# ALVI-Labs/frankenstein

Hardware: AMD Instinct MI355X
Metric: neural frames/sec (train fwd+bwd+AdamW, whole job) (higher is better)
Workload: dtype bf16; 1 GPU; brainformer-small (6L d=384 6x64 heads, N=6144 tokens) + 2-block perceiver, L1 head; fwd+bwd+clip+AdamW; per_gpu_batch=32, global_batch=32, frames_T=600, electrodes=256, parallelism=dp1, weights=random-init (seed 42)

## Files before the change

frankenstein_amd/_lib.py:

```python
from __future__ import annotations

import ctypes as C
from pathlib import Path

import os

LIB_PATH = Path(os.environ.get("FRANKEN_HIP_LIB") or Path(__file__).resolve().parent / "libfranken_hip.so")

FK_F32, FK_BF16 = 0, 1
MASK_NONE, MASK_CAUSAL, MASK_BLOCK_CAUSAL, MASK_PREFIX, MASK_KEYPAD, MASK_DENSE = 0, 1, 2, 3, 4, 5
NORM_LAYER, NORM_RMS = 0, 1
ATTN_Q_PRESCALED = 1
GEMV_GELU = 1
NT_RING2, NT_RING192, NT_RING128, NT_BIG, NT_GLDS4, NT_GLDS, NT_STAGED = range(7)
NT_ROUTE_F32 = -2
ATTN_FWD_GENERIC, ATTN_FWD_FEWQ, ATTN_FWD_PS, ATTN_FWD_ASM = range(4)
ATTN_DQ_GENERIC, ATTN_DQ_FEWQ, ATTN_DQ_PS, ATTN_DQ_ASM = range(4)
ATTN_DKDV_GENERIC, ATTN_DKDV_PS, ATTN_DKDV_ASM, ATTN_DKDVW_ASM = range(4)

_p, _i64, _int, _f32, _f64, _sz, _u32 = C.c_void_p, C.c_int64, C.c_int, C.c_float, C.c_double, C.c_size_t, C.c_uint32

SIGNATURES = {
    "fk_version": (_int, []),
    "fk_last_error": (C.c_char_p, []),
    "fk_gemm_nt": (_int, [_p, _i64, _p, _i64, _p, _i64, _i64, _i64, _i64, _p, _p, _i64, _i64, _int, _int, _p]),
    "fk_gemv_nt": (_int, [_p, _i64, _p, _i64, _p, _i64, _i64, _i64, _i64, _p, _p, _i64, _p, _p, _f32, _int, _int, _int, _p]),
    "fk_gemm_nt_rope": (_int, [_p, _i64, _p, _i64, _p, _i64, _i64, _i64, _i64, _p, _p, _i64, _i64, _i64, _i64, _i64, _i64, _i64, _int, _p]),
    "fk_gemm_nt_swiglu": (_int, [_p, _i64, _p, _i64, _p, _i64, _p, _i64, _i64, _i64, _i64, _int, _p]),
    "fk_gemm_nt_dswiglu": (_int, [_p, _i64, _p, _i64, _p, _i64, _p, _i64, _i64, _i64, _i64, _int, _p]),
    "fk_mlp_bwd_fused": (_int, [_p, _i64, _p, _i64, _p, _i64, _p, _i64, _p, _i64, _p, _i64, _i64, _i64, _i64, _int, _p]),
    "fk_gemm_nt_route": (_int, [_i64, _i64, _i64, _int, _int, _int, _int]),
    "fk_gemm_tn_route": (_int, [_i64, _i64, _i64, _int, _p, _p]),
    "fk_gemm_tn_workspace_bytes": (_sz, [_i64, _i64, _i64, _int]),
    "fk_gemm_tn": (_int, [_p, _i64, _p, _i64, _p, _i64, _i64, _i64, _i64, _int, _int, _p, _sz, _p]),
    "fk_gemm_tn_swiglu": (_int, [_p, _i64, _p, _i64, _p, _p, _i64, _i64, _i64, _i64, _int, _p, _sz, _p]),
    "fk_colsum_workspace_bytes": (_sz, [_i64, _i64]),
    "fk_colsum": (_int, [_p, _i64, _p, _i64, _i64, _int, _int, _p, _sz, _p]),
    "fk_attn_fwd": (_int, [_p, _p, _p, _p, _p] + [_i64] * 13 + [_int, _i64, _i64, _i64, _p, _p, _f32, _int, _int, _p]),
    "fk_attn_bwd": (_int, [_p] * 10 + [_i64] * 13 + [_int, _i64, _i64, _i64, _p, _p, _f32, _p, _i64, _i64, _int, _int, _p]),
    "fk_attn_fwd_dropout": (_int, [_p, _p, _p, _p, _p] + [_i64] * 13 + [_int, _i64, _i64, _i64, _p, _p, _f32, _int, _f32, _p, _u32, _int, _p]),
    "fk_attn_bwd_dropout": (_int, [_p] * 10 + [_i64] * 13 + [_int, _i64, _i64, _i64, _p, _p, _f32, _p, _i64, _i64, _int, _f32, _p, _u32, _int, _p]),
    "fk_attn_route": (_int, [_i64, _i64, _i64, _int, _int, _i64, _i64, _i64, _int, _int, _int, _p, _p, _p]),
    "fk_dropout": (_int, [_p, _p, _p, _i64, _f32, _p, _u32, _int, _p]),
    "fk_norm_fwd": (_int, [_p, _p, _p, _p, _p, _p, _i64, _i64, _f32, _int, _int, _p]),
    "fk_norm_bwd_workspace_bytes": (_sz, [_i64, _i64]),
    "fk_norm_bwd": (_int, [_p] * 9 + [_i64, _i64, _int, _int, _int, _p, _sz, _p]),
    "fk_rope": (_int, [_p, _i64, _i64, _i64, _i64, _i64, _p, _i64, _i64, _int, _int, _p]),
    "fk_patchify": (_int, [_p, _p, _i64, _i64, _i64, _i64, _i64, _int, _p]),
    "fk_swiglu_fwd": (_int, [_p, _p, _i64, _i64, _int, _p]),
    "fk_swiglu_bwd": (_int, [_p, _p, _p, _i64, _i64, _int, _p]),
    "fk_gelu_fwd": (_int, [_p, _p, _i64, _int, _p]),
    "fk_gelu_bwd": (_int, [_p, _p, _p, _i64, _int, _p]),
    "fk_cast_pack": (_int, [_p, _i64, _p, _i64, _i64, _i64, _int, _int, _p]),
    "fk_cast_pack_rows": (_int, [_p, _i64, _p, _i64, _i64, _i64, _int, _i64, _i64, _i64, _int, _p]),
    "fk_cast_pack_multi": (_int, [_p, _i64, _i64, _int, _p]),
    "fk_cast": (_int, [_p, _int, _p, _int, _i64, _p]),
    "fk_add": (_int, [_p, _p, _p, _i64, _int, _p]),
    "fk_gather_rows": (_int, [_p, _i64, _int, _p, _i64, _p, _i64, _int, _i64, _i64, _i64, _int, _p]),
    "fk_scatter_add_rows": (_int, [_p, _int, _p, _i64, _p, _i64, _i64, _p]),
    "fk_prefix_mask": (_int, [_p, _p, _i64, _p, _p, _i64, _i64, _i64, _p]),
    "fk_copy2d": (_int, [_p, _i64, _p, _i64, _i64, _i64, _int, _p]),
    "fk_attn_combine": (_int, [_p, _p, _p, _p, _i64, _i64, _i64, _i64, _i64, _int, _p]),
    "fk_add2d": (_int, [_p, _i64, _p, _i64, _i64, _i64, _p]),
    "fk_gpt_embed_step": (_int, [_p, _p, _p, _p, _p, _i64, _i64, _i64, _int, _p]),
    "fk_kv_append": (_int, [_p, _p, _p, _i64, _i64, _i64, _int, _p]),
    "fk_attn_decode": (_int, [_p, _i64, _p, _i64, _i64, _p, _i64, _p, _i64, _i64, _i64, _f32, _int, _p]),
    "fk_sample_topk": (_int, [_p, _i64, _i64, _i64, _f32, _i64, _p, _p, _p, _p, _p, _i64, _i64, _p, _p]),
    "fk_attn_decode_beam": (_int, [_p, _i64, _p, _i64, _i64, _p, _i64, _p, _i64, _p, _i64, _i64, _i64, _f32, _int, _p]),
    "fk_beam_topk": (_int, [_p, _i64, _i64, _i64, _f32, _i64, _p, _p, _p]),
    "fk_beam_select": (_int, [_p, _p, _i64, _i64, _i64, _p, _p, _p, _p, _p, _p, _p, _p, _i64, _p, _i64, _p]),
    "fk_attn_decode_beam_grouped": (_int, [_p, _i64, _p, _i64, _i64, _i64, _p, _i64, _p, _i64, _p, _i64, _i64, _i64, _i64, _f32, _int, _int, _p]),
    "fk_beam_select_grouped": (_int, [_p, _p, _i64, _i64, _i64, _i64, _i64, _p, _p, _p, _p, _p, _p, _p, _p, _i64, _p, _i64, _p, _p]),
    "fk_beam_select_eos": (_int, [_p, _p, _i64, _i64, _i64, _i64, _i64, _p, _p, _p, _p, _p, _p, _p, _p, _i64, _p, _i64, _p, _i64, _p, _p, _p, _i64, _p, _p, _p]),
    "fk_beam_backtrack": (_int, [_p, _p, _i64, _i64, _i64, _p, _p, _p, _p, _i64, _p, _i64, _i64, _i64, _i64, _p, _p, _p]),
    "fk_sample_topk_eos": (_int, [_p, _i64, _i64, _i64, _f32, _i64, _p, _p, _p, _p, _p, _i64, _i64, _p, _i64, _p, _p, _p, _p, _p]),
# ... 82 lines not shown
```

frankenstein_amd/csrc/attention.hip:

```cpp
#include "fk_common.h"
#include <type_traits>

namespace {

constexpr int NT = 256;
constexpr int BQ = 128;
constexpr int BKV = 64;
constexpr float LOG2E = 1.4426950408889634f;

struct AttnArgs {
  const void *Q, *K, *V, *O, *dO;
  void *Out, *dQ, *dK, *dV;
  float *LSE, *delta;
  int64_t q_bs, q_rs, k_bs, k_rs, v_bs, v_rs, o_bs, o_rs;
  int B, H, Nq, Nk;
  int mask_kind, mask_c, q_off, k_off;
  float scale;
  const float* rope_table; int64_t rope_bs; int rope_off;
  const int* limits; const int* qfirst;
  int flags;
  const unsigned* drop_seed; unsigned drop_site, drop_thresh; float drop_scale;
};

template <typename T, int D> struct AT {
// ... 696 lines not shown
    }
    const char* kt = buf + (i & 1) * FEWQ_TILE;
    const char* vt = kt + FEWQ_BK * 128;
    const int kb = (wave + FEWQ_NW * i) * FEWQ_BK;
    f32x16 sc, dp;
#pragma unroll
    for (int r = 0; r < 16; ++r) { sc[r] = 0.0f; dp[r] = 0.0f; }
#pragma unroll
    for (int s = 0; s < 4; ++s) {
      Frag<T> kf, vf;
      img_row<T, D>(kf, kt, li, s, lh);
      img_row<T, D>(vf, vt, li, s, lh);
      mma32<T>(sc, kf, qf[s]);
      mma32<T>(dp, vf, gf[s]);
    }
    const bool ragged = kb + FEWQ_BK > p.Nk;
#pragma unroll
    for (int r = 0; r < 16; ++r) {
      float pv = __builtin_amdgcn_exp2f(sc[r] * c - lse2);
      if (ragged && kb + acc_row(r, lh) >= p.Nk) pv = 0.0f;
      sc[r] = pv * (dp[r] - dl);
    }
#pragma unroll
    for (int s = 0; s < 2; ++s) {
      Frag<T> df;
      frag_from_acc<T>(df, sc, s);
#pragma unroll
      for (int dt = 0; dt < 2; ++dt) {
        Frag<T> ktf;
        img_tr<T, D>(ktf, kt, 0, s, 32 * dt, lane);
        mma32<T>(dq[dt], ktf, df);
      }
    }
  }
  __syncthreads();
  float* area = reinterpret_cast<float*>(smem);
  {
    float* mine = area + wave * 32 * 64;
#pragma unroll
    for (int dt = 0; dt < 2; ++dt)
#pragma unroll
      for (int r = 0; r < 16; ++r) mine[(dt * 16 + r) * 64 + lane] = dq[dt][r];
  }
  __syncthreads();
  if (wave != 0) return;
#pragma unroll 1
  for (int w = 1; w < FEWQ_NW; ++w) {
    const float* theirs = area + w * 32 * 64;
#pragma unroll
    for (int dt = 0; dt < 2; ++dt)
#pragma unroll
      for (int r = 0; r < 16; ++r) dq[dt][r] += theirs[(dt * 16 + r) * 64 + lane];
  }
  T* dQp = head_ptr<T, D>(p.dQ, p.q_bs, b, hd);
  store_rows_T<T, D>(dQp, p.q_rs, qrow, q_ok, dq, p.scale, lh);
}

template <bool DMA> FK_DEV void tile_sync() {
  if constexpr (DMA) asm volatile("s_waitcnt vmcnt(0) lgkmcnt(0)\n\ts_barrier" ::: "memory");
  else __syncthreads();
}
template <typename T, int D>
__global__ __launch_bounds__(NT) void attn_bwd_dq_kernel(AttnArgs p) {
  using C = AT<T, D>;
  extern __shared__ __attribute__((aligned(16))) char smem[];
  constexpr int IMG = BKV * C::RSTRIDE;
// ... 1482 lines not shown
                        float drop_p, const uint32_t* drop_seed, uint32_t drop_site, int dtype, void* stream) {
  const int64_t st[8] = {q_bs, q_rs, k_bs, k_rs, v_bs, v_rs, o_bs, o_rs};
  int rc = check_common("fk_attn_bwd", B, H, Nq, Nk, D, dtype, mask_kind, mask_c, st, 8);
  if (rc) return rc;
  rc = check_flags_tables("fk_attn_bwd", D, dtype, mask_kind, q_off, k_off, limits, qfirst, flags);
  if (rc) return rc;
  FK_CHECK_ARG(Q && K && V && O && dO && LSE && dQ && dK && dV && delta_ws, "fk_attn_bwd: null pointer");
  FK_CHECK_ARG((((uintptr_t)Q | (uintptr_t)K | (uintptr_t)V | (uintptr_t)O | (uintptr_t)dO | (uintptr_t)dQ | (uintptr_t)dK | (uintptr_t)dV) & 15) == 0,
               "fk_attn_bwd: pointers must be 16-byte aligned");
  AttnArgs a{};
  a.Q = Q; a.K = K; a.V = V; a.O = O; a.dO = dO; a.LSE = const_cast<float*>(LSE); a.delta = delta_ws;
  a.dQ = dQ; a.dK = dK; a.dV = dV;
  fill_common(a, st, B, H, Nq, Nk, mask_kind, mask_c, q_off, k_off, limits, qfirst, scale, flags);
  FK_CHECK_ARG(!rope_table || (Nq == Nk && D % 4 == 0 && ((uintptr_t)rope_table & 15) == 0), "fk_attn_bwd: fused inverse RoPE needs self-attention (Nq == Nk)");
  a.rope_table = rope_table; a.rope_bs = rope_bs; a.rope_off = (int)rope_off;
  rc = set_dropout("fk_attn_bwd", a, drop_p, drop_seed, drop_site, flags);
  if (rc) return rc;
  FK_ATTN_DISPATCH(launch_bwd, a, (hipStream_t)stream);
  FK_CHECK_LAUNCH("fk_attn_bwd");
  return FK_OK;
}

int fk_attn_bwd(const void* Q, const void* K, const void* V, const void* O, const void* dO, const float* LSE,
                void* dQ, void* dK, void* dV, float* delta_ws, int64_t B, int64_t H, int64_t Nq, int64_t Nk, int64_t D,
                int64_t q_bs, int64_t q_rs, int64_t k_bs, int64_t k_rs, int64_t v_bs, int64_t v_rs, int64_t o_bs,
                int64_t o_rs, int mask_kind, int64_t mask_c, int64_t q_off, int64_t k_off, const int32_t* limits,
                const int32_t* qfirst, float scale, const float* rope_table, int64_t rope_bs, int64_t rope_off, int flags,
                int dtype, void* stream) {
  return fk_attn_bwd_dropout(Q, K, V, O, dO, LSE, dQ, dK, dV, delta_ws, B, H, Nq, Nk, D, q_bs, q_rs, k_bs, k_rs, v_bs, v_rs, o_bs, o_rs,
                             mask_kind, mask_c, q_off, k_off, limits, qfirst, scale, rope_table, rope_bs, rope_off, flags, 0.0f, nullptr, 0,
                             dtype, stream);
}

int fk_attn_route(int64_t Nq, int64_t Nk, int64_t D, int dtype, int mask_kind, int64_t mask_c, int64_t q_off, int64_t k_off, int flags,
                  int has_dropout, int has_rope, int* fwd, int* dq, int* dkdv) {
  const int64_t st[1] = {0};
  int rc = check_common("fk_attn_route", 1, 1, Nq, Nk, D, dtype, mask_kind, mask_c, st, 0);
  if (rc) return rc;
  FK_CHECK_ARG((flags & ~FK_ATTN_Q_PRESCALED) == 0 && (!(flags & FK_ATTN_Q_PRESCALED) || (dtype == FK_BF16 && D == 64)),
               "fk_attn_route: bad flags %d (FK_ATTN_Q_PRESCALED needs bf16, D = 64)", flags);
  FK_CHECK_ARG(!(flags & FK_ATTN_Q_PRESCALED) || (mask_kind != FK_MASK_DENSE && !has_dropout),
               "fk_attn_route: dense masks and dropout run on the generic kernels (no FK_ATTN_Q_PRESCALED)");
  FK_CHECK_ARG(!has_rope || Nq == Nk, "fk_attn_route: fused inverse RoPE needs self-attention (Nq == Nk)");
  AttnArgs a{};
  a.Nq = (int)Nq; a.Nk = (int)Nk; a.mask_kind = mask_kind; a.mask_c = (int)mask_c; a.q_off = (int)q_off; a.k_off = (int)k_off;
  a.flags = flags; a.drop_thresh = has_dropout ? 1u : 0u;
  static_assert(Img<bf16_t, 64>::SWZ && !Img<bf16_t, 32>::SWZ && !Img<bf16_t, 128>::SWZ && !Img<float, 64>::SWZ, "the swizzled image: bf16, D = 64");
  const AttnRoute r = attn_route(a, dtype == FK_BF16 && D == 64, has_rope != 0);
  if (fwd) *fwd = r.fwd;
  if (dq) *dq = r.dq;
  if (dkdv) *dkdv = r.dkdv;
  return FK_OK;
}

}
```

frankenstein_amd/engine.py:

```python
from __future__ import annotations

from typing import List, Optional, Sequence, Tuple

import math
import os
import weakref

import torch

from . import kernels as K
from .kernels import NO_MASK

Tensor = torch.Tensor

_COMPUTE_DTYPE = torch.bfloat16
_EPOCH = 0


def set_compute_dtype(dtype) -> None:
    global _COMPUTE_DTYPE
    if isinstance(dtype, str):
        dtype = {"bf16": torch.bfloat16, "bfloat16": torch.bfloat16, "fp32": torch.float32, "float32": torch.float32}[dtype]
    assert dtype in (torch.bfloat16, torch.float32)
    _COMPUTE_DTYPE = dtype
# ... 424 lines not shown
class CrossAttnBranch(torch.autograd.Function):

    @staticmethod
    def forward(ctx, x, context, ln_w, ln_b, qw, kw, vw, pw, spec):
        H, D, mask, eps = spec
        B, T, d = x.shape
        Nc = context.shape[1]
        HD = H * D
        x2, c2 = x.view(B * T, d), context.view(B * Nc, d)
        h, mean, rstd = K.norm_fwd(x2, ln_w.detach(), ln_b.detach(), eps)
        ctx.ln_b = ln_b
        q = K.gemm_nt(h, shadow([qw]))
        kv = K.gemm_nt(c2, shadow([kw, vw]))
        kv3 = kv.view(B, Nc, 2 * HD)
        o, lse = K.attn_fwd(q.view(B, T, H, D), kv3[..., :HD].unflatten(-1, (H, D)), kv3[..., HD:].unflatten(-1, (H, D)), mask)
        y = K.gemm_nt(o.view(B * T, HD), shadow([pw]), residual=x2)
        ctx.spec = spec
        ctx.save_for_backward(x, context, ln_w, qw, kw, vw, pw, h, mean, rstd, q, kv, o, lse)
        return y.view(B, T, d)

    @staticmethod
    def backward(ctx, dy):
        H, D, mask, eps = ctx.spec
        x, context, ln_w, qw, kw, vw, pw, h, mean, rstd, q, kv, o, lse = ctx.saved_tensors
        B, T, d = x.shape
        Nc, HD = context.shape[1], H * D
        x2, c2 = x.view(B * T, d), context.view(B * Nc, d)
        dy2 = dy.contiguous().view(B * T, d)
        do = K.gemm_nt(dy2, shadow([pw], transpose=True))
        (dpw,) = wgrad(dy2, o.view(B * T, HD), [pw])
        dkv = torch.empty_like(kv)
        dq = torch.empty_like(q)
        kv3, dkv3 = kv.view(B, Nc, 2 * HD), dkv.view(B, Nc, 2 * HD)
        K.attn_bwd(q.view(B, T, H, D), kv3[..., :HD].unflatten(-1, (H, D)), kv3[..., HD:].unflatten(-1, (H, D)), o,
                   do.view(B, T, H, D), lse, dq.view(B, T, H, D), dkv3[..., :HD].unflatten(-1, (H, D)),
                   dkv3[..., HD:].unflatten(-1, (H, D)), mask)
        dh = K.gemm_nt(dq, shadow([qw], transpose=True))
        (dqw,) = wgrad(dq, h, [qw])
        dctx = K.gemm_nt(dkv, shadow([kw, vw], transpose=True))
        dkw, dvw = wgrad(dkv, c2, [kw, vw])
        dx, dg, db = norm_bwd(dh, x2, ln_w, ctx.ln_b, mean, rstd, dres=dy2)
        return dx.view(B, T, d), dctx.view(B, Nc, d), dg, db, dqw, dkw, dvw, dpw, None


_MLP_BWD_FUSED = os.environ.get("FK_MLP_BWD_FUSED", "1") != "0"


class MlpBranch(torch.autograd.Function):

    @staticmethod
    def forward(ctx, x, ln_w, ln_b, up_w, up_b, gate_w, down_w, down_b, spec):
        residual, eps, nkind = spec[:3]
        drop = spec[3] if len(spec) > 3 else None
        shp = x.shape
        d = shp[-1]
        x2 = x.reshape(-1, d)
        has_ln = ln_w is not None
        if has_ln:
            h, mean, rstd = K.norm_fwd(x2, ln_w.detach(), None if ln_b is None else ln_b.detach(), eps, nkind)
        else:
            h, mean, rstd = x2, None, None
        fused = gate_w is not None and up_b is None and up_w.shape[0] % 8 == 0
        if fused:
            a, g = K.gemm_nt_swiglu(h, shadow_swiglu(up_w, gate_w))
        else:
            ups = [up_w] if gate_w is None else [up_w, gate_w]
            a = K.gemm_nt(h, shadow(ups), bias=None if up_b is None else shadow([up_b]))
            g = K.gelu_fwd(a) if gate_w is None else K.swiglu_fwd(a)
        if drop is None:
# ... 498 lines not shown
```

frankenstein_amd/kernels.py:

```python
from __future__ import annotations

import math
from typing import Optional, Tuple

import torch

from . import _lib
from ._lib import FK_BF16, FK_F32, MASK_BLOCK_CAUSAL, MASK_CAUSAL, MASK_DENSE, MASK_KEYPAD, MASK_NONE, MASK_PREFIX, NORM_LAYER, NORM_RMS, ATTN_Q_PRESCALED, call, lib

Tensor = torch.Tensor


TIMERS = None
TIMER_PREFIX = None


class _timed:
    __slots__ = ("name", "ev")

    def __init__(self, name):
        self.name = name

    def __enter__(self):
        self.ev = None
# ... 299 lines not shown
        call("fk_attn_fwd", q.data_ptr(), k.data_ptr(), v.data_ptr(), out.data_ptr(), lse.data_ptr(), B, H, Nq, Nk, D,
             qb, qr, kb, kr, vb, vr, ob, orr, mask.kind, mask.c, mask.q_off, mask.k_off, _ptr(mask.limits), _ptr(mask.qfirst),
             sc, ATTN_Q_PRESCALED if q_prescaled else 0, fk_dtype(q), _stream())
      else:
        call("fk_attn_fwd_dropout", q.data_ptr(), k.data_ptr(), v.data_ptr(), out.data_ptr(), lse.data_ptr(), B, H, Nq, Nk, D,
             qb, qr, kb, kr, vb, vr, ob, orr, mask.kind, mask.c, mask.q_off, mask.k_off, _ptr(mask.limits), _ptr(mask.qfirst),
             sc, ATTN_Q_PRESCALED if q_prescaled else 0, dropout[0], dropout[1].data_ptr(), dropout[2], fk_dtype(q), _stream())
    return out, lse


def attn_bwd(q: Tensor, k: Tensor, v: Tensor, o: Tensor, do: Tensor, lse: Tensor, dq: Tensor, dk: Tensor, dv: Tensor,
             mask: Mask = NO_MASK, scale: Optional[float] = None, rope_table: Optional[Tensor] = None,
             rope_off: int = 0, q_prescaled: bool = False, dropout: Optional[tuple] = None) -> None:
    B, Nq, H, D = q.shape
    Nk = k.shape[1]
    (qb, qr), (kb, kr), (vb, vr), (ob, orr) = _bnhd(q), _bnhd(k), _bnhd(v), _bnhd(o)
    assert _bnhd(dq) == (qb, qr) and _bnhd(dk) == (kb, kr) and _bnhd(dv) == (vb, vr) and _bnhd(do) == (ob, orr)
    assert do.dtype == q.dtype and dq.dtype == q.dtype
    _check_dense(mask, B, H, Nq, Nk)
    delta = torch.empty(2 * B * H * ((Nq + 63) // 64 * 64), dtype=torch.float32, device=q.device)
    sc = scale if scale is not None else 1.0 / math.sqrt(D)
    with _timed(f"attn_bwd:{B}x{H}x{Nq}x{Nk}x{D}:m{mask.kind}"):
      head = (q.data_ptr(), k.data_ptr(), v.data_ptr(), o.data_ptr(), do.data_ptr(), lse.data_ptr(),
              dq.data_ptr(), dk.data_ptr(), dv.data_ptr(), delta.data_ptr(), B, H, Nq, Nk, D, qb, qr, kb, kr, vb, vr, ob, orr,
              mask.kind, mask.c, mask.q_off, mask.k_off, _ptr(mask.limits), _ptr(mask.qfirst), sc, _ptr(rope_table),
              0 if rope_table is None or rope_table.dim() == 3 else rope_table.stride(0), rope_off,
              ATTN_Q_PRESCALED if q_prescaled else 0)
      if dropout is None:
        call("fk_attn_bwd", *head, fk_dtype(q), _stream())
      else:
        call("fk_attn_bwd_dropout", *head, dropout[0], dropout[1].data_ptr(), dropout[2], fk_dtype(q), _stream())


ATTN_FWD_ROUTE_NAMES = {_lib.ATTN_FWD_GENERIC: "FWD_GENERIC", _lib.ATTN_FWD_FEWQ: "FWD_FEWQ", _lib.ATTN_FWD_PS: "FWD_PS", _lib.ATTN_FWD_ASM: "FWD_ASM"}
ATTN_DQ_ROUTE_NAMES = {_lib.ATTN_DQ_GENERIC: "DQ_GENERIC", _lib.ATTN_DQ_FEWQ: "DQ_FEWQ", _lib.ATTN_DQ_PS: "DQ_PS", _lib.ATTN_DQ_ASM: "DQ_ASM"}
ATTN_DKDV_ROUTE_NAMES = {_lib.ATTN_DKDV_GENERIC: "DKDV_GENERIC", _lib.ATTN_DKDV_PS: "DKDV_PS", _lib.ATTN_DKDV_ASM: "DKDV_ASM", _lib.ATTN_DKDVW_ASM: "DKDVW_ASM"}


def attn_route(Nq: int, Nk: int, D: int, dtype=torch.bfloat16, mask: Mask = NO_MASK, q_prescaled: bool = False, dropout: bool = False,
               rope: bool = False) -> Tuple[int, int, int]:
    import ctypes
    f, q, kv = ctypes.c_int(-1), ctypes.c_int(-1), ctypes.c_int(-1)
    call("fk_attn_route", Nq, Nk, D, fk_dtype(dtype), mask.kind, mask.c, mask.q_off, mask.k_off, ATTN_Q_PRESCALED if q_prescaled else 0,
         int(dropout), int(rope), ctypes.byref(f), ctypes.byref(q), ctypes.byref(kv))
    return f.value, q.value, kv.value


def attn_route_names(*args, **kw) -> Tuple[str, str, str]:
    f, q, kv = attn_route(*args, **kw)
    return ATTN_FWD_ROUTE_NAMES[f], ATTN_DQ_ROUTE_NAMES[q], ATTN_DKDV_ROUTE_NAMES[kv]


def attn_combine(parts: Tensor, lse_parts: Optional[Tensor] = None, want_lse: bool = True):
    B, S, T, H, D = parts.shape
    assert parts.is_contiguous()
    out = torch.empty((B, T, H, D), dtype=parts.dtype, device=parts.device)
    lse = None
    if lse_parts is not None:
        assert lse_parts.dtype == torch.float32 and lse_parts.is_contiguous() and lse_parts.shape == (B, S, H, T)
        lse = torch.empty((B, H, T), dtype=torch.float32, device=parts.device) if want_lse else None
    call("fk_attn_combine", parts.data_ptr(), _ptr(lse_parts), out.data_ptr(), _ptr(lse), B, S, T, H, D, fk_dtype(parts), _stream())
    return out, lse


def norm_fwd(x: Tensor, gamma: Tensor, beta: Optional[Tensor], eps: float, kind: int = NORM_LAYER):
    x2 = _as2d(x)
# ... 825 lines not shown
```

include/franken_hip.h:

```cpp
#ifndef FRANKEN_HIP_H
#define FRANKEN_HIP_H

#include <stddef.h>
#include <stdint.h>

#ifdef __cplusplus
extern "C" {
#endif

#define FK_VERSION 302

#define FK_OK 0
#define FK_EINVAL (-1)
#define FK_ELAUNCH (-2)
#define FK_EUNSUPPORTED (-3)

enum { FK_F32 = 0, FK_BF16 = 1 };
enum { FK_MASK_NONE = 0, FK_MASK_CAUSAL = 1, FK_MASK_BLOCK_CAUSAL = 2, FK_MASK_PREFIX = 3, FK_MASK_KEYPAD = 4, FK_MASK_DENSE = 5 };
enum { FK_ATTN_Q_PRESCALED = 1 };
enum { FK_NORM_LAYER = 0, FK_NORM_RMS = 1 };
enum { FK_ACT_SWIGLU = 0, FK_ACT_GELU = 1 };
enum { FK_GEMV_GELU = 1 };

int fk_version(void);
// ... 25 lines not shown
                      int64_t H, int64_t N2, int dtype, void* workspace, size_t workspace_bytes, void* stream);
int fk_gemm_tn_route(int64_t M, int64_t N1, int64_t N2, int dtype, int* nsplit, int64_t* rows_per_split);
size_t fk_colsum_workspace_bytes(int64_t rows, int64_t cols);
int fk_colsum(const void* X, int64_t ld, float* out, int64_t rows, int64_t cols, int accumulate, int dtype,
              void* workspace, size_t workspace_bytes, void* stream);

int fk_attn_fwd(const void* Q, const void* K, const void* V, void* O, float* LSE, int64_t B, int64_t H, int64_t Nq,
                int64_t Nk, int64_t D, int64_t q_bs, int64_t q_rs, int64_t k_bs, int64_t k_rs, int64_t v_bs,
                int64_t v_rs, int64_t o_bs, int64_t o_rs, int mask_kind, int64_t mask_c, int64_t q_off, int64_t k_off,
                const int32_t* limits, const int32_t* qfirst, float scale, int flags, int dtype, void* stream);
int fk_attn_bwd(const void* Q, const void* K, const void* V, const void* O, const void* dO, const float* LSE,
                void* dQ, void* dK, void* dV, float* delta_ws, int64_t B, int64_t H, int64_t Nq, int64_t Nk, int64_t D,
                int64_t q_bs, int64_t q_rs, int64_t k_bs, int64_t k_rs, int64_t v_bs, int64_t v_rs, int64_t o_bs,
                int64_t o_rs, int mask_kind, int64_t mask_c, int64_t q_off, int64_t k_off, const int32_t* limits,
                const int32_t* qfirst, float scale, const float* rope_table, int64_t rope_bs, int64_t rope_off, int flags,
                int dtype, void* stream);

int fk_attn_fwd_dropout(const void* Q, const void* K, const void* V, void* O, float* LSE, int64_t B, int64_t H, int64_t Nq,
                        int64_t Nk, int64_t D, int64_t q_bs, int64_t q_rs, int64_t k_bs, int64_t k_rs, int64_t v_bs,
                        int64_t v_rs, int64_t o_bs, int64_t o_rs, int mask_kind, int64_t mask_c, int64_t q_off, int64_t k_off,
                        const int32_t* limits, const int32_t* qfirst, float scale, int flags, float drop_p, const uint32_t* drop_seed,
                        uint32_t drop_site, int dtype, void* stream);
int fk_attn_bwd_dropout(const void* Q, const void* K, const void* V, const void* O, const void* dO, const float* LSE,
                        void* dQ, void* dK, void* dV, float* delta_ws, int64_t B, int64_t H, int64_t Nq, int64_t Nk, int64_t D,
                        int64_t q_bs, int64_t q_rs, int64_t k_bs, int64_t k_rs, int64_t v_bs, int64_t v_rs, int64_t o_bs,
                        int64_t o_rs, int mask_kind, int64_t mask_c, int64_t q_off, int64_t k_off, const int32_t* limits,
                        const int32_t* qfirst, float scale, const float* rope_table, int64_t rope_bs, int64_t rope_off, int flags,
                        float drop_p, const uint32_t* drop_seed, uint32_t drop_site, int dtype, void* stream);
enum { FK_ATTN_FWD_GENERIC = 0, FK_ATTN_FWD_FEWQ = 1, FK_ATTN_FWD_PS = 2, FK_ATTN_FWD_ASM = 3 };
enum { FK_ATTN_DQ_GENERIC = 0, FK_ATTN_DQ_FEWQ = 1, FK_ATTN_DQ_PS = 2, FK_ATTN_DQ_ASM = 3 };
enum { FK_ATTN_DKDV_GENERIC = 0, FK_ATTN_DKDV_PS = 1, FK_ATTN_DKDV_ASM = 2, FK_ATTN_DKDVW_ASM = 3 };
int fk_attn_route(int64_t Nq, int64_t Nk, int64_t D, int dtype, int mask_kind, int64_t mask_c, int64_t q_off, int64_t k_off, int flags,
                  int has_dropout, int has_rope, int* fwd, int* dq, int* dkdv);

int fk_dropout(const void* x, const void* res, void* y, int64_t n, float p, const uint32_t* seed, uint32_t site, int dtype, void* stream);

int fk_norm_fwd(const void* x, const float* gamma, const float* beta, void* y, float* mean, float* rstd,
                int64_t rows, int64_t dim, float eps, int kind, int dtype, void* stream);
size_t fk_norm_bwd_workspace_bytes(int64_t rows, int64_t dim);
int fk_norm_bwd(const void* dy, const void* x, const float* gamma, const float* mean, const float* rstd,
                const void* dres, void* dx, float* dgamma, float* dbeta, int64_t rows, int64_t dim, int kind,
                int accumulate, int dtype, void* workspace, size_t workspace_bytes, void* stream);

int fk_rope(void* x, int64_t B, int64_t T, int64_t ld, int64_t nheads, int64_t D, const float* table, int64_t table_bs,
            int64_t pos_off, int conj, int dtype, void* stream);

int fk_patchify(const float* x, void* tok, int64_t B, int64_t T, int64_t C, int64_t P, int64_t ldp, int dtype,
                void* stream);

int fk_swiglu_fwd(const void* h13, void* g, int64_t rows, int64_t H, int dtype, void* stream);
int fk_swiglu_bwd(const void* h13, const void* dg, void* dh13, int64_t rows, int64_t H, int dtype, void* stream);
int fk_gelu_fwd(const void* x, void* y, int64_t n, int dtype, void* stream);
int fk_gelu_bwd(const void* x, const void* dy, void* dx, int64_t n, int dtype, void* stream);

int fk_cast_pack(const float* src, int64_t lds, void* dst, int64_t ldd, int64_t rows, int64_t cols, int transpose,
                 int dtype, void* stream);
int fk_cast_pack_rows(const float* src, int64_t lds, void* dst, int64_t ldd, int64_t rows, int64_t cols, int transpose,
                      int64_t rblk, int64_t rstride, int64_t roff, int dtype, void* stream);
typedef struct fk_pack_job {
  const float* src; void* dst; int64_t lds, ldd;
  int32_t rows, cols, transpose, rblk, rstride, roff;
  int64_t chunk_begin;
} fk_pack_job;
int fk_cast_pack_multi(const fk_pack_job* jobs, int64_t njobs, int64_t total_chunks, int dtype, void* stream);
int fk_cast(const void* src, int src_dtype, void* dst, int dst_dtype, int64_t n, void* stream);
int fk_add(const void* a, const void* b, void* y, int64_t n, int dtype, void* stream);
// ... 152 lines not shown
```

Baseline: 406,700 frames/s.

## Add fused few-query attention backward computing dQ, dK, dV in one kernel

Adds a bf16, head-dim-64 attention backward kernel for the perceiver cross-attention, where there are few queries and many keys. Each block handles one batch-head. It keeps Q and dO in registers, double-buffers K/V tiles through LDS, and computes dQ, dK and dV in a single pass. This replaces the separate delta, dQ and dK/dV launches and their repeated K/V reads. The cost is the scores being recomputed in two orientations per tile, plus new hand-written LDS transpose reads and counted waits.

```diff
diff --git a/frankenstein_amd/_lib.py b/frankenstein_amd/_lib.py
--- a/frankenstein_amd/_lib.py
+++ b/frankenstein_amd/_lib.py
@@ -41,6 +41,8 @@
     "fk_attn_fwd_dropout": (_int, [_p, _p, _p, _p, _p] + [_i64] * 13 + [_int, _i64, _i64, _i64, _p, _p, _f32, _int, _f32, _p, _u32, _int, _p]),
     "fk_attn_bwd_dropout": (_int, [_p] * 10 + [_i64] * 13 + [_int, _i64, _i64, _i64, _p, _p, _f32, _p, _i64, _i64, _int, _f32, _p, _u32, _int, _p]),
     "fk_attn_route": (_int, [_i64, _i64, _i64, _int, _int, _i64, _i64, _i64, _int, _int, _int, _p, _p, _p]),
+    "fk_attn_bwd_fewq_ok": (_int, [_i64, _i64, _i64, _int, _int]),
+    "fk_attn_bwd_fewq": (_int, [_p] * 9 + [_i64] * 13 + [_int, _f32, _int, _p]),
     "fk_dropout": (_int, [_p, _p, _p, _i64, _f32, _p, _u32, _int, _p]),
     "fk_norm_fwd": (_int, [_p, _p, _p, _p, _p, _p, _i64, _i64, _f32, _int, _int, _p]),
     "fk_norm_bwd_workspace_bytes": (_sz, [_i64, _i64]),
diff --git a/frankenstein_amd/csrc/attention.hip b/frankenstein_amd/csrc/attention.hip
--- a/frankenstein_amd/csrc/attention.hip
+++ b/frankenstein_amd/csrc/attention.hip
@@ -752,6 +752,222 @@
         mma32<T>(dq[dt], ktf, df);
       }
     }
+  }
+  __syncthreads();
+  float* area = reinterpret_cast<float*>(smem);
+  {
+    float* mine = area + wave * 32 * 64;
+#pragma unroll
+    for (int dt = 0; dt < 2; ++dt)
+#pragma unroll
+      for (int r = 0; r < 16; ++r) mine[(dt * 16 + r) * 64 + lane] = dq[dt][r];
+  }
+  __syncthreads();
+  if (wave != 0) return;
+#pragma unroll 1
+  for (int w = 1; w < FEWQ_NW; ++w) {
+    const float* theirs = area + w * 32 * 64;
+#pragma unroll
+    for (int dt = 0; dt < 2; ++dt)
+#pragma unroll
+      for (int r = 0; r < 16; ++r) dq[dt][r] += theirs[(dt * 16 + r) * 64 + lane];
+  }
+  T* dQp = head_ptr<T, D>(p.dQ, p.q_bs, b, hd);
+  store_rows_T<T, D>(dQp, p.q_rs, qrow, q_ok, dq, p.scale, lh);
+}
+
+constexpr int FEWQ_ROW_STORES = 8;
+FK_DEV void fewq_ktr(Frag<bf16_t> (&f)[2][2], const char* img, int lane) {
+  const int g = lane >> 4, i = lane & 15, h = g >> 1;
+  typedef unsigned u32x2_t __attribute__((ext_vector_type(2)));
+  unsigned a[2][2][2];
+  u32x2_t r[2][2][2];
+#pragma unroll
+  for (int s = 0; s < 2; ++s)
+#pragma unroll
+    for (int dt = 0; dt < 2; ++dt)
+#pragma unroll
+      for (int t = 0; t < 2; ++t) {
+        const int row = 16 * s + 8 * t + 4 * h + (i >> 2), col = 32 * dt + 16 * (g & 1) + 4 * (i & 3);
+        a[s][dt][t] = (unsigned)(uintptr_t)(lds_void_t*)(img + Img<bf16_t, 64>::off(row, col * 2));
+      }
+  asm volatile(
+      "ds_read_b64_tr_b16 %0, %8\n\tds_read_b64_tr_b16 %1, %9\n\tds_read_b64_tr_b16 %2, %10\n\tds_read_b64_tr_b16 %3, %11\n\t"
+      "ds_read_b64_tr_b16 %4, %12\n\tds_read_b64_tr_b16 %5, %13\n\tds_read_b64_tr_b16 %6, %14\n\tds_read_b64_tr_b16 %7, %15\n\t"
+      "s_waitcnt lgkmcnt(0)"
+      : "=&v"(r[0][0][0]), "=&v"(r[0][0][1]), "=&v"(r[0][1][0]), "=&v"(r[0][1][1]), "=&v"(r[1][0][0]), "=&v"(r[1][0][1]), "=&v"(r[1][1][0]),
+        "=&v"(r[1][1][1])
+      : "v"(a[0][0][0]), "v"(a[0][0][1]), "v"(a[0][1][0]), "v"(a[0][1][1]), "v"(a[1][0][0]), "v"(a[1][0][1]), "v"(a[1][1][0]), "v"(a[1][1][1])
+      : "memory");
+#pragma unroll
+  for (int s = 0; s < 2; ++s)
+#pragma unroll
+    for (int dt = 0; dt < 2; ++dt)
+#pragma unroll
+      for (int t = 0; t < 2; ++t) {
+        const bf16x4 v = __builtin_bit_cast(bf16x4, r[s][dt][t]);
+#pragma unroll
+        for (int e = 0; e < 4; ++e) f[s][dt].v[4 * t + e] = v[e];
+      }
+}
+FK_DEV void fewq_store_tile(bf16_t* base, int64_t rs, int row0, int nrows, const f32x16 (&acc)[2], float mul, char* img, int lane) {
+  typedef unsigned u32x2_t __attribute__((ext_vector_type(2)));
+  const int li = lane & 31, lh = lane >> 5;
+#pragma unroll
+  for (int dt = 0; dt < 2; ++dt)
+#pragma unroll
+    for (int g = 0; g < 4; ++g) {
+      const u32x2_t v = {pack_bf16x2(acc[dt][4 * g] * mul, acc[dt][4 * g + 1] * mul), pack_bf16x2(acc[dt][4 * g + 2] * mul, acc[dt][4 * g + 3] * mul)};
+      *reinterpret_cast<u32x2_t*>(img + Img<bf16_t, 64>::off(li, (32 * dt + 8 * g + 4 * lh) * 2)) = v;
+    }
+#pragma unroll
+  for (int j = 0; j < 4; ++j) {
+    const int r = 8 * j + (lane >> 3), row = row0 + r;
+    const u32x4 v = *reinterpret_cast<const u32x4*>(img + Img<bf16_t, 64>::off(r, (lane & 7) * 16));
+    if (row < nrows) fk_st<FK_NT_STORES_ATTN != 0>(reinterpret_cast<u32x4*>(base + (int64_t)row * rs + (lane & 7) * 8), v);
+  }
+}
+
+__global__ __launch_bounds__(FEWQ_NW * 64) void attn_bwd_fewq_kernel(AttnArgs p) {
+  using T = bf16_t;
+  constexpr int D = 64;
+  extern __shared__ __attribute__((aligned(16))) char smem[];
+  const int tid = threadIdx.x, lane = tid & 63, li = lane & 31, lh = lane >> 5;
+  const int wave = __builtin_amdgcn_readfirstlane(tid >> 6);
+  const int bh = blockIdx.x, b = bh / p.H, hd = bh % p.H;
+  const T* Qp = head_ptr<T, D>(p.Q, p.q_bs, b, hd);
+  const T* Kp = head_ptr<T, D>(p.K, p.k_bs, b, hd);
+  const T* Vp = head_ptr<T, D>(p.V, p.v_bs, b, hd);
+  const T* Gp = head_ptr<T, D>(p.dO, p.o_bs, b, hd);
+  const T* Op = head_ptr<T, D>(p.O, p.o_bs, b, hd);
+  T* dKp = head_ptr<T, D>(p.dK, p.k_bs, b, hd);
+  T* dVp = head_ptr<T, D>(p.dV, p.v_bs, b, hd);
+  const int qrow = li;
+  const bool q_ok = qrow < p.Nq;
+  Frag<T> qf[4], gf[4];
+  float part = 0.0f;
+#pragma unroll
+  for (int s = 0; s < 4; ++s) {
+    if (q_ok) {
+      frag_load_contig<T>(qf[s], Qp + (int64_t)qrow * p.q_rs + 16 * s + 8 * lh);
+      frag_load_contig<T>(gf[s], Gp + (int64_t)qrow * p.o_rs + 16 * s + 8 * lh);
+      Frag<T> of;
+      frag_load_contig<T>(of, Op + (int64_t)qrow * p.o_rs + 16 * s + 8 * lh);
+#pragma unroll
+      for (int e = 0; e < 8; ++e) part += to_f32<T>(of.v[e]) * to_f32<T>(gf[s].v[e]);
+    } else {
+      frag_zero<T>(qf[s]);
+      frag_zero<T>(gf[s]);
+    }
+  }
+  const int64_t stat = ((int64_t)b * p.H + hd) * p.Nq + qrow;
+  const float lse2 = q_ok ? p.LSE[stat] * LOG2E : INFINITY;
+  const float dl = part + __shfl_xor(part, 32, 64);
+  char* buf = smem + wave * 2 * FEWQ_TILE;
+  const int ntiles = (p.Nk + FEWQ_BK - 1) / FEWQ_BK;
+  const int cnt = wave < ntiles ? (ntiles - wave + FEWQ_NW - 1) / FEWQ_NW : 0;
+  float lse_r[16], dl_r[16];
+#pragma unroll
+  for (int r = 0; r < 16; ++r) {
+    lse_r[r] = __shfl(lse2, acc_row(r, lh), 64);
+    dl_r[r] = __shfl(dl, acc_row(r, lh), 64);
+  }
+  Frag<T> qt[2][2], gt[2][2];
+  {
+    char* qi = buf + FEWQ_TILE;
+    char* gi = qi + FEWQ_BK * 128;
+#pragma unroll
+    for (int s = 0; s < 4; ++s) {
+      *reinterpret_cast<bf16x8*>(qi + Img<T, D>::off(li, (16 * s + 8 * lh) * 2)) = qf[s].v;
+      *reinterpret_cast<bf16x8*>(gi + Img<T, D>::off(li, (16 * s + 8 * lh) * 2)) = gf[s].v;
+    }
+#pragma unroll
+    for (int s = 0; s < 2; ++s)
+#pragma unroll
+      for (int dt = 0; dt < 2; ++dt) {
+        img_tr<T, D>(qt[s][dt], qi, 0, s, 32 * dt, lane);
+        img_tr<T, D>(gt[s][dt], gi, 0, s, 32 * dt, lane);
+      }
+  }
+  asm volatile("s_waitcnt vmcnt(0) lgkmcnt(0)" ::: "memory");
+  auto request = [&](int i) __attribute__((always_inline)) {
+    char* img = buf + (i & 1) * FEWQ_TILE;
+    const int row0 = (wave + FEWQ_NW * i) * FEWQ_BK;
+    dma_tile_bf16_d64<FEWQ_BK, 1>(Kp, p.k_rs, row0, p.Nk, img, 0, lane);
+    dma_tile_bf16_d64<FEWQ_BK, 1>(Vp, p.v_rs, row0, p.Nk, img + FEWQ_BK * 128, 0, lane);
+  };
+  if (cnt > 0) request(0);
+  const float c = p.scale * LOG2E;
+  f32x16 dq[2];
+  zero_acc(dq);
+  for (int i = 0; i < cnt; ++i) {
+    if (i + 1 < cnt) {
+      request(i + 1);
+      static_assert(FEWQ_ROW_STORES == 8, "the counted waits below");
+      if (i == 0) asm volatile("s_waitcnt vmcnt(8)" ::: "memory");
+      else asm volatile("s_waitcnt vmcnt(16)" ::: "memory");
+    } else {
+      asm volatile("s_waitcnt vmcnt(0)" ::: "memory");
+    }
+    const char* kt = buf + (i & 1) * FEWQ_TILE;
+    const char* vt = kt + FEWQ_BK * 128;
+    const int kb = (wave + FEWQ_NW * i) * FEWQ_BK;
+    Frag<T> kf[4], vf[4];
+    f32x16 sc, dp;
+#pragma unroll
+    for (int r = 0; r < 16; ++r) { sc[r] = 0.0f; dp[r] = 0.0f; }
+#pragma unroll
+    for (int s = 0; s < 4; ++s) {
+      img_row<T, D>(kf[s], kt, li, s, lh);
+      img_row<T, D>(vf[s], vt, li, s, lh);
+      mma32<T>(sc, kf[s], qf[s]);
+      mma32<T>(dp, vf[s], gf[s]);
+    }
+    const bool ragged = kb + FEWQ_BK > p.Nk;
+#pragma unroll
+    for (int r = 0; r < 16; ++r) {
+      float pv = __builtin_amdgcn_exp2f(sc[r] * c - lse2);
+      if (ragged && kb + acc_row(r, lh) >= p.Nk) pv = 0.0f;
+      sc[r] = pv * (dp[r] - dl);
+    }
+    Frag<T> ktf[2][2];
+    fewq_ktr(ktf, kt, lane);
+#pragma unroll
+    for (int s = 0; s < 2; ++s) {
+      Frag<T> df;
+      frag_from_acc<T>(df, sc, s);
+#pragma unroll
+      for (int dt = 0; dt < 2; ++dt) mma32<T>(dq[dt], ktf[s][dt], df);
+    }
+#pragma unroll
+    for (int r = 0; r < 16; ++r) { sc[r] = 0.0f; dp[r] = 0.0f; }
+#pragma unroll
+    for (int s = 0; s < 4; ++s) {
+      mma32<T>(sc, qf[s], kf[s]);
+      mma32<T>(dp, gf[s], vf[s]);
+    }
+#pragma unroll
+    for (int r = 0; r < 16; ++r) {
+      const float pv = __builtin_amdgcn_exp2f(sc[r] * c - lse_r[r]);
+      sc[r] = pv;
+      dp[r] = pv * (dp[r] - dl_r[r]);
+    }
+    f32x16 dk[2], dv[2];
+    zero_acc(dk);
+    zero_acc(dv);
+#pragma unroll
+    for (int s = 0; s < 2; ++s) {
+      Frag<T> pf, df;
+      frag_from_acc<T>(pf, sc, s);
+      frag_from_acc<T>(df, dp, s);
+#pragma unroll
+      for (int dt = 0; dt < 2; ++dt) {
+        mma32<T>(dv[dt], gt[s][dt], pf);
+        mma32<T>(dk[dt], qt[s][dt], df);
+      }
+    }
+    fewq_store_tile(dKp, p.k_rs, kb, p.Nk, dk, p.scale, const_cast<char*>(kt), lane);
+    fewq_store_tile(dVp, p.v_rs, kb, p.Nk, dv, 1.0f, const_cast<char*>(vt), lane);
   }
   __syncthreads();
   float* area = reinterpret_cast<float*>(smem);
@@ -2300,6 +2516,34 @@
                              dtype, stream);
 }
 
+int fk_attn_bwd_fewq_ok(int64_t Nq, int64_t Nk, int64_t D, int dtype, int mask_kind) {
+  if (Nq < 1 || Nk >= (1LL << 30)) return 0;
+  AttnArgs a{};
+  a.Nq = (int)Nq; a.Nk = (int)Nk; a.mask_kind = mask_kind;
+  return dtype == FK_BF16 && D == 64 && few_queries(a);
+}
+
+int fk_attn_bwd_fewq(const void* Q, const void* K, const void* V, const void* O, const void* dO, const float* LSE,
+                     void* dQ, void* dK, void* dV, int64_t B, int64_t H, int64_t Nq, int64_t Nk, int64_t D,
+                     int64_t q_bs, int64_t q_rs, int64_t k_bs, int64_t k_rs, int64_t v_bs, int64_t v_rs, int64_t o_bs,
+                     int64_t o_rs, int mask_kind, float scale, int dtype, void* stream) {
+  const int64_t st[8] = {q_bs, q_rs, k_bs, k_rs, v_bs, v_rs, o_bs, o_rs};
+  int rc = check_common("fk_attn_bwd_fewq", B, H, Nq, Nk, D, dtype, mask_kind, 0, st, 8);
+  if (rc) return rc;
+  FK_CHECK_ARG(fk_attn_bwd_fewq_ok(Nq, Nk, D, dtype, mask_kind),
+               "fk_attn_bwd_fewq: needs bf16, head_dim 64, Nq <= 32, Nk >= 1024 and no mask (fk_attn_bwd_fewq_ok); fk_attn_bwd takes the rest");
+  FK_CHECK_ARG(Q && K && V && O && dO && LSE && dQ && dK && dV, "fk_attn_bwd_fewq: null pointer");
+  FK_CHECK_ARG((((uintptr_t)Q | (uintptr_t)K | (uintptr_t)V | (uintptr_t)O | (uintptr_t)dO | (uintptr_t)dQ | (uintptr_t)dK | (uintptr_t)dV) & 15) == 0,
+               "fk_attn_bwd_fewq: pointers must be 16-byte aligned");
+  AttnArgs a{};
+  a.Q = Q; a.K = K; a.V = V; a.O = O; a.dO = dO; a.LSE = const_cast<float*>(LSE);
+  a.dQ = dQ; a.dK = dK; a.dV = dV;
+  fill_common(a, st, B, H, Nq, Nk, mask_kind, 0, 0, 0, nullptr, nullptr, scale, 0);
+  launch_attn<attn_bwd_fewq_kernel>((unsigned)(a.H * a.B), FEWQ_NW * 64, FEWQ_LDS, (hipStream_t)stream, a);
+  FK_CHECK_LAUNCH("fk_attn_bwd_fewq");
+  return FK_OK;
+}
+
 int fk_attn_route(int64_t Nq, int64_t Nk, int64_t D, int dtype, int mask_kind, int64_t mask_c, int64_t q_off, int64_t k_off, int flags,
                   int has_dropout, int has_rope, int* fwd, int* dq, int* dkdv) {
   const int64_t st[1] = {0};
diff --git a/frankenstein_amd/engine.py b/frankenstein_amd/engine.py
--- a/frankenstein_amd/engine.py
+++ b/frankenstein_amd/engine.py
@@ -480,9 +480,10 @@
         dkv = torch.empty_like(kv)
         dq = torch.empty_like(q)
         kv3, dkv3 = kv.view(B, Nc, 2 * HD), dkv.view(B, Nc, 2 * HD)
-        K.attn_bwd(q.view(B, T, H, D), kv3[..., :HD].unflatten(-1, (H, D)), kv3[..., HD:].unflatten(-1, (H, D)), o,
-                   do.view(B, T, H, D), lse, dq.view(B, T, H, D), dkv3[..., :HD].unflatten(-1, (H, D)),
-                   dkv3[..., HD:].unflatten(-1, (H, D)), mask)
+        q4, k4 = q.view(B, T, H, D), kv3[..., :HD].unflatten(-1, (H, D))
+        bwd = K.attn_bwd_fewq if K.attn_bwd_fewq_ok(q4, k4, mask) else K.attn_bwd
+        bwd(q4, k4, kv3[..., HD:].unflatten(-1, (H, D)), o, do.view(B, T, H, D), lse, dq.view(B, T, H, D),
+            dkv3[..., :HD].unflatten(-1, (H, D)), dkv3[..., HD:].unflatten(-1, (H, D)), mask)
         dh = K.gemm_nt(dq, shadow([qw], transpose=True))
         (dqw,) = wgrad(dq, h, [qw])
         dctx = K.gemm_nt(dkv, shadow([kw, vw], transpose=True))
diff --git a/frankenstein_amd/kernels.py b/frankenstein_amd/kernels.py
--- a/frankenstein_amd/kernels.py
+++ b/frankenstein_amd/kernels.py
@@ -355,6 +355,26 @@
         call("fk_attn_bwd_dropout", *head, dropout[0], dropout[1].data_ptr(), dropout[2], fk_dtype(q), _stream())
 
 
+def attn_bwd_fewq_ok(q: Tensor, k: Tensor, mask: Mask = NO_MASK) -> bool:
+    if q.dtype not in (torch.bfloat16, torch.float32):
+        return False
+    return bool(lib().fk_attn_bwd_fewq_ok(q.shape[1], k.shape[1], q.shape[3], fk_dtype(q), mask.kind))
+
+
+def attn_bwd_fewq(q: Tensor, k: Tensor, v: Tensor, o: Tensor, do: Tensor, lse: Tensor, dq: Tensor, dk: Tensor, dv: Tensor,
+                  mask: Mask = NO_MASK, scale: Optional[float] = None) -> None:
+    B, Nq, H, D = q.shape
+    Nk = k.shape[1]
+    (qb, qr), (kb, kr), (vb, vr), (ob, orr) = _bnhd(q), _bnhd(k), _bnhd(v), _bnhd(o)
+    assert _bnhd(dq) == (qb, qr) and _bnhd(dk) == (kb, kr) and _bnhd(dv) == (vb, vr) and _bnhd(do) == (ob, orr)
+    assert do.dtype == q.dtype and dq.dtype == q.dtype and k.dtype == q.dtype and v.dtype == q.dtype
+    sc = scale if scale is not None else 1.0 / math.sqrt(D)
+    with _timed(f"attn_bwd_fewq:{B}x{H}x{Nq}x{Nk}x{D}"):
+        call("fk_attn_bwd_fewq", q.data_ptr(), k.data_ptr(), v.data_ptr(), o.data_ptr(), do.data_ptr(), lse.data_ptr(),
+             dq.data_ptr(), dk.data_ptr(), dv.data_ptr(), B, H, Nq, Nk, D, qb, qr, kb, kr, vb, vr, ob, orr, mask.kind, sc,
+             fk_dtype(q), _stream())
+
+
 ATTN_FWD_ROUTE_NAMES = {_lib.ATTN_FWD_GENERIC: "FWD_GENERIC", _lib.ATTN_FWD_FEWQ: "FWD_FEWQ", _lib.ATTN_FWD_PS: "FWD_PS", _lib.ATTN_FWD_ASM: "FWD_ASM"}
 ATTN_DQ_ROUTE_NAMES = {_lib.ATTN_DQ_GENERIC: "DQ_GENERIC", _lib.ATTN_DQ_FEWQ: "DQ_FEWQ", _lib.ATTN_DQ_PS: "DQ_PS", _lib.ATTN_DQ_ASM: "DQ_ASM"}
 ATTN_DKDV_ROUTE_NAMES = {_lib.ATTN_DKDV_GENERIC: "DKDV_GENERIC", _lib.ATTN_DKDV_PS: "DKDV_PS", _lib.ATTN_DKDV_ASM: "DKDV_ASM", _lib.ATTN_DKDVW_ASM: "DKDVW_ASM"}
diff --git a/include/franken_hip.h b/include/franken_hip.h
--- a/include/franken_hip.h
+++ b/include/franken_hip.h
@@ -81,6 +81,11 @@
 enum { FK_ATTN_DKDV_GENERIC = 0, FK_ATTN_DKDV_PS = 1, FK_ATTN_DKDV_ASM = 2, FK_ATTN_DKDVW_ASM = 3 };
 int fk_attn_route(int64_t Nq, int64_t Nk, int64_t D, int dtype, int mask_kind, int64_t mask_c, int64_t q_off, int64_t k_off, int flags,
                   int has_dropout, int has_rope, int* fwd, int* dq, int* dkdv);
+int fk_attn_bwd_fewq_ok(int64_t Nq, int64_t Nk, int64_t D, int dtype, int mask_kind);
+int fk_attn_bwd_fewq(const void* Q, const void* K, const void* V, const void* O, const void* dO, const float* LSE,
+                     void* dQ, void* dK, void* dV, int64_t B, int64_t H, int64_t Nq, int64_t Nk, int64_t D,
+                     int64_t q_bs, int64_t q_rs, int64_t k_bs, int64_t k_rs, int64_t v_bs, int64_t v_rs, int64_t o_bs,
+                     int64_t o_rs, int mask_kind, float scale, int dtype, void* stream);
 
 int fk_dropout(const void* x, const void* res, void* y, int64_t n, float p, const uint32_t* seed, uint32_t site, int dtype, void* stream);
 
```

After: 408,800 frames/s (median of 6 runs). No clear change (+0.5%).
